# xianlopez/optical_flow

Measured on AMD Instinct MI355X. Metric: image-pairs/sec training, 384x512 batch=8 per GPU, higher is better.
Workload: dtype fp32

## Files before the change

optical_flow_amd/csrc/conv_f32.hip:

```cpp
#include "common.h"
#include "conv_dev.h"
#include "conv_narrow.h"

#include <algorithm>

namespace oflow {

template <int BM, int BN, int WAVES_M, int WAVES_N, int MODE>
__global__ __launch_bounds__(256, 2) void conv_gemm_f32(GemmArgs a) {
  constexpr int WM = BM / WAVES_M, WN = BN / WAVES_N;
  constexpr int TM = WM / 32, TN = WN / 32;
  static_assert(WAVES_M * WAVES_N == 4, "4 waves");
  static_assert(TM >= 1 && TN >= 1 && WM % 32 == 0 && WN % 32 == 0, "tile");
  constexpr bool A_KCONTIG = (MODE != MODE_WGRAD);
  constexpr int SA = BM + 4;
  constexpr int SB = BN + 4;
  constexpr int A_SLOTS = BM * BK / 4 / 256;
  constexpr int B_QUADS = BK * BN / 4;
  constexpr int B_SLOTS = (B_QUADS + 255) / 256;
  static_assert(A_SLOTS >= 1, "BM >= 64");

  static_assert(2 * BK * (SA + SB) >= 4 * 1024, "epilogue images fit LDS");
  __shared__ float smem[2 * BK * (SA + SB)];
  float (*As)[BK * SA] = reinterpret_cast<float (*)[BK * SA]>(smem);
// ... 2859 lines not shown
    const int trem = t - b * tiles_x * tiles_y;
    const int oy0 = (trem / tiles_x) * XH, ox0 = (trem % tiles_x) * TT_W;
    const int iy0 = oy0 - a.pt, ix00 = ox0 - a.pl;
#pragma unroll
    for (int j = 0; j < XS; ++j) {
      const int q = tid + NT * j;
      const int r2 = q / (CIB / 4);
      const int half = r2 & 1, s = (r2 >> 1) % KS, hy = (r2 >> 1) / KS;
      const int iy = iy0 + hy;
      const bool rok = q < XQ && xc_ok && (unsigned)iy < (unsigned)a.h;
      const int ix0 = ix00 + 8 * half + s;
      const int base = ((b * a.h + iy) * a.w + ix0) * a.lda + ci0 + 4 * xcq;
#pragma unroll
      for (int e = 0; e < 8; ++e) {
        const bool ok = rok && (unsigned)(ix0 + e) < (unsigned)a.w;
        xv[j][e] = bload4(rx, ok ? (uint32_t)((base + e * a.lda) * 4) : kOOB);
      }
    }
  };
  auto store_x = [&]() {
#pragma unroll
    for (int j = 0; j < XS; ++j) {
      const int q = tid + NT * j;
      if (q < XQ) {
        const int r2 = q / (CIB / 4);
        const int half = r2 & 1, s = (r2 >> 1) % KS, hy = (r2 >> 1) / KS;
        const int ci = 4 * xcq;
        uint4* blk = &Xs[(s * HH + hy) * CIB * 2];
#pragma unroll
        for (int c = 0; c < 4; ++c) {
          float v8[8];
#pragma unroll
          for (int e = 0; e < 8; ++e) v8[e] = (&xv[j][e].x)[c];
          bf16x8 h, m, l;
          split3x8(v8, h, m, l);
          const int idx = xrow(ci + c) * 2 + (half ^ xoct(ci + c));
          blk[idx] = __builtin_bit_cast(uint4, h);
          blk[PL + idx] = __builtin_bit_cast(uint4, m);
          blk[2 * PL + idx] = __builtin_bit_cast(uint4, l);
        }
      }
    }
  };
  const int co = co0 + wco0 + lrow;
  const bool co_ok = co < a.nb;
  const uint32_t dy_lane = (uint32_t)((8 * lk * a.ldb + co) * 4);
  const bool dy_co_full = co0 + COB <= a.nb;
  auto load_dy = [&](float (&dv)[8], int t, int kk) {
    const int b = t / (tiles_x * tiles_y);
    const int trem = t - b * tiles_x * tiles_y;
    const int oy = (trem / tiles_x) * XH + kk, ox0 = (trem % tiles_x) * TT_W;
    if (dy_co_full && oy < a.ho && ox0 + TT_W <= a.wo) {
      const int so = ((b * a.ho + oy) * a.wo + ox0) * a.ldb * 4;
#pragma unroll
      for (int e = 0; e < 8; ++e)
        dv[e] = __builtin_bit_cast(float, __builtin_amdgcn_raw_buffer_load_b32(
                                              rd, dy_lane + e * a.ldb * 4, so, 0));
      return;
    }
    const int ox = ox0 + 8 * lk;
    const bool rok = co_ok && oy < a.ho;
    const int base = ((b * a.ho + oy) * a.wo + ox) * a.ldb + co;
#pragma unroll
    for (int e = 0; e < 8; ++e) {
      const bool ok = rok && ox + e < a.wo;
      dv[e] = bload1(rd, ok ? (uint32_t)((base + e * a.ldb) * 4) : kOOB);
    }
  };

  f32x16 acc[KS];
#pragma unroll
  for (int t = 0; t < KS; ++t)
#pragma unroll
    for (int r = 0; r < 16; ++r) acc[t][r] = 0.f;
  const int a_base = xrow(wci0 + lrow) * 2 + (lk ^ xoct(wci0 + lrow));
  float colacc = 0.f;
  float dcur[8], dnext[8];

  if (steps > 0) {
    load_x(t_begin);
    load_dy(dcur, t_begin, 0);
    store_x();
  }
  __syncthreads();
  for (int i = 0; i < steps; ++i) {
    const int t = t_begin + i;
    const bool more = i + 1 < steps;
    if (more) load_x(t + 1);
#pragma unroll
    for (int kk = 0; kk < XH; ++kk) {
      if (kk + 1 < XH) load_dy(dnext, t, kk + 1);
      else if (more) load_dy(dnext, t + 1, 0);
      __builtin_amdgcn_sched_barrier(0);
      bf16x8 bh, bm, bl;
      split3x8(dcur, bh, bm, bl);
      if (do_colsum) {
#pragma unroll
        for (int e = 0; e < 8; ++e) colacc += dcur[e];
      }
      bf16x8 fa[2][NP];
      auto load_a = [&](bf16x8 (&f)[NP], int s) {
        const int xa = (s * HH + kk + wr) * CIB * 2 + a_base;
#pragma unroll
        for (int p = 0; p < NP; ++p) f[p] = __builtin_bit_cast(bf16x8, Xs[p * PL + xa]);
      };
      load_a(fa[0], 0);
#pragma unroll
      for (int s = 0; s < KS; ++s) {
          if (s + 1 < KS) load_a(fa[(s + 1) & 1], s + 1);
          __builtin_amdgcn_sched_barrier(0);
          const bf16x8 ah = fa[s & 1][0], am = fa[s & 1][1], al = fa[s & 1][2];
          f32x16 x = acc[s];
          x = __builtin_amdgcn_mfma_f32_32x32x16_bf16(al, bh, x, 0, 0, 0);
          x = __builtin_amdgcn_mfma_f32_32x32x16_bf16(ah, bl, x, 0, 0, 0);
          x = __builtin_amdgcn_mfma_f32_32x32x16_bf16(am, bm, x, 0, 0, 0);
          x = __builtin_amdgcn_mfma_f32_32x32x16_bf16(am, bh, x, 0, 0, 0);
          x = __builtin_amdgcn_mfma_f32_32x32x16_bf16(ah, bm, x, 0, 0, 0);
          acc[s] = __builtin_amdgcn_mfma_f32_32x32x16_bf16(ah, bh, x, 0, 0, 0);
          __builtin_amdgcn_sched_barrier(0);
      }
#pragma unroll
      for (int e = 0; e < 8; ++e) dcur[e] = dnext[e];
    }
    __syncthreads();
    if (more) store_x();
    __syncthreads();
  }

  float* S = a.slab + (int64_t)split * a.split_stride;
  if (do_colsum) {
    const float v = colacc + __shfl_xor(colacc, 32);
    if (lk == 0 && co < a.N) S[(int64_t)a.M * a.slab_ld + co] = v;
  }
  if (co < a.N) {
#pragma unroll
    for (int s = 0; s < KS; ++s)
#pragma unroll
      for (int r = 0; r < 16; ++r) {
        const int ci = ci0 + wci0 + (r & 3) + 8 * (r >> 2) + 4 * lk;
        if (ci < a.kc) S[((int64_t)(wr * KS + s) * a.kc + ci) * a.slab_ld + co] = acc[s][r];
      }
  }
}

__device__ __forceinline__ int wgx3b_slot(int ci, int oct) {
  return (ci >> 3) * 16 + ((2 * (ci & 7) + oct) ^ (((ci >> 3) & 3) << 1));
}

template <int CIB>
__device__ __forceinline__ int wgx3b_sw(int hx) {
  return ((hx >> 3) & 1) | (CIB == 64 ? ((hx >> 1) & 1) << 1 : 0);
}

template <int WAVES_CI, int WAVES_CO, int XH, int MI, int NP, int STG>
__device__ __forceinline__ void wgrad_x3b_body(const GemmArgs& a) {
  constexpr int NJ = 2 / MI;
  static_assert(MI * NJ == 2, "18 accumulator tiles per wave");
  static_assert(NP == 1 || NP == 3, "planes");
  static_assert(STG == 0 || STG == 1, "staging: three shifted copies / one pixel-major image");
  constexpr int NT = 64 * WAVES_CI * WAVES_CO;
  constexpr int CIB = 16 * MI * WAVES_CI, COB = 16 * NJ * WAVES_CO, KS = 3, HH = XH + KS - 1;
  static_assert(XH % 2 == 0 && (CIB == 32 || CIB == 64), "k-steps of 2 tile rows; wgx3b_sw");
  constexpr int HW = TT_W + KS - 1;
  constexpr int XQ = STG ? HH * HW * (CIB / 4) : HH * KS * 2 * (CIB / 4), XS = (XQ + NT - 1) / NT;
  constexpr int RB = CIB * 2;
  constexpr int PL = KS * HH * RB;
  constexpr int PXB = CIB * 2;
  constexpr int PLB = HH * HW * PXB, IMGB = NP * PLB;
  constexpr int LDSB = STG ? 2 * IMGB : NP * PL * 16;
  static_assert(NT / 64 * 512 * 4 <= LDSB && LDSB % 16 == 0, "epilogue images fit LDS");
  __shared__ uint4 Xs[LDSB / 16];
  char* const xlds = reinterpret_cast<char*>(Xs);

  const int tid = threadIdx.x;
  const int lane = tid & 63;
  const int wave = __builtin_amdgcn_readfirstlane(tid >> 6);
  const int wgid = xcd_remap(blockIdx.x, gridDim.x);
  const int split = wgid / a.tiles_total;
  const int tile = wgid - split * a.tiles_total;
  const int tile_co = tile % a.n_tiles;
  const int tile_ci = tile / a.n_tiles;
  const int ci0 = tile_ci * CIB, co0 = tile_co * COB;
  const int t_begin = split * a.k_per_split;
  const int t_end = min(a.K, t_begin + a.k_per_split);
  const int steps = max(0, t_end - t_begin);
  const int tiles_x = (a.wo + TT_W - 1) / TT_W, tiles_y = (a.ho + XH - 1) / XH;
  const rsrc_t rx = make_rsrc(a.A, a.a_bytes);
  const rsrc_t rd = make_rsrc(a.B, a.b_bytes);
  const int wci0 = (wave / WAVES_CO) * 16 * MI;
  const int wco0 = (wave % WAVES_CO) * 16 * NJ;
  const int l16 = lane & 15, lq = lane >> 4;

  const int xcq = tid % (CIB / 4);
  const bool xc_ok = ci0 + 4 * xcq < a.kc;
  constexpr int XE = STG ? 1 : 8;
  float4 xv[XS][XE];
  auto load_x = [&](int t) {
    const int b = t / (tiles_x * tiles_y);
    const int trem = t - b * tiles_x * tiles_y;
    const int oy0 = (trem / tiles_x) * XH, ox0 = (trem % tiles_x) * TT_W;
    const int iy0 = oy0 - a.pt, ix00 = ox0 - a.pl;
#pragma unroll
    for (int j = 0; j < XS; ++j) {
      const int q = tid + NT * j;
      if constexpr (STG == 1) {
        const int hp = q / (CIB / 4);
        const int hy = hp / HW, hx = hp - hy * HW;
        const int iy = iy0 + hy, ix = ix00 + hx;
        const bool ok = q < XQ && xc_ok && (unsigned)iy < (unsigned)a.h &&
                        (unsigned)ix < (unsigned)a.w;
        const int base = ((b * a.h + iy) * a.w + ix) * a.lda + ci0 + 4 * xcq;
        xv[j][0] = bload4(rx, ok ? (uint32_t)(base * 4) : kOOB);
      } else {
        const int r2 = q / (CIB / 4);
        const int half = r2 & 1, s = (r2 >> 1) % KS, hy = (r2 >> 1) / KS;
        const int iy = iy0 + hy;
        const bool rok = q < XQ && xc_ok && (unsigned)iy < (unsigned)a.h;
        const int ix0 = ix00 + 8 * half + s;
        const int base = ((b * a.h + iy) * a.w + ix0) * a.lda + ci0 + 4 * xcq;
#pragma unroll
        for (int e = 0; e < 8; ++e) {
          const bool ok = rok && (unsigned)(ix0 + e) < (unsigned)a.w;
          xv[j][e] = bload4(rx, ok ? (uint32_t)((base + e * a.lda) * 4) : kOOB);
        }
      }
    }
  };
  auto store_x = [&](int j, int buf) {
    const int q = tid + NT * j;
    if (XQ % NT == 0 || q < XQ) {
      if constexpr (STG == 1) {
        const int hp = q / (CIB / 4);
        const int hx = hp % HW;
        char* dst = xlds + buf * IMGB + hp * PXB + (((xcq >> 2) ^ wgx3b_sw<CIB>(hx)) << 5) +
                    8 * (xcq & 3);
        if constexpr (NP == 1) {
          *reinterpret_cast<uint2*>(dst) = pack_bf16x4(xv[j][0]);
        } else {
          uint2 h, m, l;
          split3x4(xv[j][0], h, m, l);
          *reinterpret_cast<uint2*>(dst) = h;
          *reinterpret_cast<uint2*>(dst + PLB) = m;
          *reinterpret_cast<uint2*>(dst + 2 * PLB) = l;
        }
      } else {
        const int r2 = q / (CIB / 4);
        const int half = r2 & 1, s = (r2 >> 1) % KS, hy = (r2 >> 1) / KS;
        uint4* blk = &Xs[(s * HH + hy) * RB];
#pragma unroll
        for (int c = 0; c < 4; ++c) {
          float v8[8];
#pragma unroll
          for (int e = 0; e < 8; ++e) v8[e] = (&xv[j][e].x)[c];
          const int idx = wgx3b_slot(4 * xcq + c, half);
          if constexpr (NP == 1) {
            blk[idx] = pack_bf16x8(make_float4(v8[0], v8[1], v8[2], v8[3]),
                                   make_float4(v8[4], v8[5], v8[6], v8[7]));
          } else {
            bf16x8 h, m, l;
            split3x8(v8, h, m, l);
            blk[idx] = __builtin_bit_cast(uint4, h);
            blk[PL + idx] = __builtin_bit_cast(uint4, m);
            blk[2 * PL + idx] = __builtin_bit_cast(uint4, l);
          }
        }
      }
    }
  };
  auto store_x_all = [&](int buf) {
#pragma unroll
    for (int j = 0; j < XS; ++j) store_x(j, buf);
  };
  int co[NJ];
  bool co_ok[NJ];
#pragma unroll
  for (int j = 0; j < NJ; ++j) {
    co[j] = co0 + wco0 + 16 * j + l16;
    co_ok[j] = co[j] < a.nb;
  }
  const int prow = lq >> 1, pcol = 8 * (lq & 1);
  const bool dy_co_full = co0 + COB <= a.nb;
  const uint32_t dy_lane = (uint32_t)(((prow * a.wo + pcol) * a.ldb + co0 + wco0 + l16) * 4);
  auto load_dy = [&](float (&dv)[NJ][8], int t, int kk) {
    const int b = t / (tiles_x * tiles_y);
    const int trem = t - b * tiles_x * tiles_y;
    const int oyr = (trem / tiles_x) * XH + 2 * kk, ox0 = (trem % tiles_x) * TT_W;
    if (dy_co_full && oyr + 1 < a.ho && ox0 + TT_W <= a.wo) {
      const int so = ((b * a.ho + oyr) * a.wo + ox0) * a.ldb * 4;
#pragma unroll
      for (int j = 0; j < NJ; ++j)
#pragma unroll
        for (int e = 0; e < 8; ++e)
          dv[j][e] = __builtin_bit_cast(float, __builtin_amdgcn_raw_buffer_load_b32(
                                                   rd, dy_lane + (e * a.ldb + 16 * j) * 4, so, 0));
      return;
    }
    const int oy = oyr + prow, ox = ox0 + pcol;
    const bool rok = oy < a.ho;
#pragma unroll
    for (int j = 0; j < NJ; ++j) {
      const int base = ((b * a.ho + oy) * a.wo + ox) * a.ldb + co[j];
#pragma unroll
      for (int e = 0; e < 8; ++e) {
        const bool ok = rok && co_ok[j] && ox + e < a.wo;
        dv[j][e] = bload1(rd, ok ? (uint32_t)((base + e * a.ldb) * 4) : kOOB);
      }
    }
  };

  f32x4 acc[KS * KS][MI][NJ];
#pragma unroll
  for (int t = 0; t < KS * KS; ++t)
#pragma unroll
    for (int i = 0; i < MI; ++i)
#pragma unroll
      for (int j = 0; j < NJ; ++j)
#pragma unroll
        for (int r = 0; r < 4; ++r) acc[t][i][j][r] = 0.f;
  int a_lane[MI];
#pragma unroll
  for (int i = 0; i < MI; ++i) a_lane[i] = prow * RB + wgx3b_slot(wci0 + 16 * i + l16, lq & 1);
  int a_tr[KS][2][MI];
  if constexpr (STG == 1) {
#pragma unroll
    for (int s = 0; s < KS; ++s)
#pragma unroll
      for (int h = 0; h < 2; ++h)
#pragma unroll
        for (int i = 0; i < MI; ++i) {
          const int hx = pcol + s + 4 * h + ((lane >> 2) & 3);
          a_tr[s][h][i] = (prow * HW + hx) * PXB +
                          ((((wci0 >> 4) + i) ^ wgx3b_sw<CIB>(hx)) << 5) + 8 * (lane & 3);
        }
  }
  const bool do_colsum = a.colsum && tile_ci == 0 && wci0 == 0;
  float colacc[NJ];
#pragma unroll
  for (int j = 0; j < NJ; ++j) colacc[j] = 0.f;
  float dcur[NJ][8], dnext[NJ][8];

  if (steps > 0) {
    load_x(t_begin);
    load_dy(dcur, t_begin, 0);
    store_x_all(0);
  }
  __syncthreads();
  for (int i = 0; i < steps; ++i) {
    const int t = t_begin + i;
    const bool more = i + 1 < steps;
    if (more) load_x(t + 1);
    const int buf = STG ? i & 1 : 0;
    int a_cur[KS][2][MI];
    if constexpr (STG == 1) {
#pragma unroll
      for (int s = 0; s < KS; ++s)
#pragma unroll
        for (int h = 0; h < 2; ++h)
#pragma unroll
          for (int ii = 0; ii < MI; ++ii) a_cur[s][h][ii] = a_tr[s][h][ii] + buf * IMGB;
    }
#pragma unroll
    for (int kk = 0; kk < XH / 2; ++kk) {
      if (kk + 1 < XH / 2) load_dy(dnext, t, kk + 1);
      else if (more) load_dy(dnext, t + 1, 0);
      __builtin_amdgcn_sched_barrier(0);
      bf16x8 bh[NJ], bm[NJ], bl[NJ];
#pragma unroll
      for (int j = 0; j < NJ; ++j) {
        if constexpr (NP == 1)
          bh[j] = __builtin_bit_cast(bf16x8, pack_bf16x8(make_float4(dcur[j][0], dcur[j][1], dcur[j][2], dcur[j][3]),
                                                         make_float4(dcur[j][4], dcur[j][5], dcur[j][6], dcur[j][7])));
        else
          split3x8(dcur[j], bh[j], bm[j], bl[j]);
      }
      if (do_colsum) {
#pragma unroll
        for (int j = 0; j < NJ; ++j)
#pragma unroll
          for (int e = 0; e < 8; ++e) colacc[j] += dcur[j][e];
      }
      bf16x8 fa[2][MI][NP];
      auto load_a = [&](bf16x8 (&f)[MI][NP], int tap) {
        const int r = tap / KS, s = tap % KS;
#pragma unroll
        for (int i = 0; i < MI; ++i) {
          if constexpr (STG == 1) {
#pragma unroll
            for (int p = 0; p < NP; ++p) {
              const int ro = p * PLB + (2 * kk + r) * HW * PXB;
              f[i][p] = tr_frag(xlds, a_cur[s][0][i] + ro, a_cur[s][1][i] + ro);
            }
          } else {
            const int xa = (s * HH + 2 * kk + r) * RB + a_lane[i];
#pragma unroll
            for (int p = 0; p < NP; ++p) f[i][p] = __builtin_bit_cast(bf16x8, Xs[p * PL + xa]);
          }
        }
      };
      load_a(fa[0], 0);
#pragma unroll
      for (int tap = 0; tap < KS * KS; ++tap) {
        if (tap + 1 < KS * KS) load_a(fa[(tap + 1) & 1], tap + 1);
        __builtin_amdgcn_sched_barrier(0);
#pragma unroll
        for (int i = 0; i < MI; ++i) {
          if constexpr (NP == 1) {
#pragma unroll
            for (int j = 0; j < NJ; ++j)
              acc[tap][i][j] = __builtin_amdgcn_mfma_f32_16x16x32_bf16(fa[tap & 1][i][0], bh[j],
                                                                       acc[tap][i][j], 0, 0, 0);
            continue;
          } else {
          const bf16x8 ah = fa[tap & 1][i][0], am = fa[tap & 1][i][1], al = fa[tap & 1][i][2];
#pragma unroll
          for (int j = 0; j < NJ; ++j) {
            f32x4 x = acc[tap][i][j];
            x = __builtin_amdgcn_mfma_f32_16x16x32_bf16(al, bh[j], x, 0, 0, 0);
            x = __builtin_amdgcn_mfma_f32_16x16x32_bf16(ah, bl[j], x, 0, 0, 0);
            x = __builtin_amdgcn_mfma_f32_16x16x32_bf16(am, bm[j], x, 0, 0, 0);
            x = __builtin_amdgcn_mfma_f32_16x16x32_bf16(am, bh[j], x, 0, 0, 0);
            x = __builtin_amdgcn_mfma_f32_16x16x32_bf16(ah, bm[j], x, 0, 0, 0);
            acc[tap][i][j] = __builtin_amdgcn_mfma_f32_16x16x32_bf16(ah, bh[j], x, 0, 0, 0);
          }
          }
        }
        __builtin_amdgcn_sched_barrier(0);
      }
#pragma unroll
      for (int j = 0; j < NJ; ++j)
#pragma unroll
        for (int e = 0; e < 8; ++e) dcur[j][e] = dnext[j][e];
      if constexpr (STG == 1) {
        if (more) {
#pragma unroll
          for (int j = 0; j < XS; ++j)
            if (j * (XH / 2) / XS == kk) store_x(j, buf ^ 1);
        }
        __builtin_amdgcn_sched_barrier(0);
      }
    }
    __syncthreads();
    if constexpr (STG == 0) {
      if (more) store_x_all(0);
      __syncthreads();
    }
  }

  float* S = a.slab + (int64_t)split * a.split_stride;
  if (do_colsum) {
#pragma unroll
    for (int j = 0; j < NJ; ++j) {
      float v = colacc[j] + __shfl_xor(colacc[j], 16);
      v += __shfl_xor(v, 32);
      if (lq == 0 && co[j] < a.N) S[(int64_t)a.M * a.slab_ld + co[j]] = v;
    }
  }
  constexpr int EW = 16 * NJ, LPR = 4 * NJ, RPI = 64 / LPR;
  float* E = reinterpret_cast<float*>(Xs) + wave * 512;
  const int c4 = lane % LPR, rr = lane / LPR;
  const bool vec = a.vec_ep;
#pragma unroll
  for (int tap = 0; tap < KS * KS; ++tap) {
    if (vec) {
#pragma unroll
      for (int i = 0; i < MI; ++i)
#pragma unroll
        for (int j = 0; j < NJ; ++j)
#pragma unroll
          for (int r = 0; r < 4; ++r) E[(16 * i + 4 * lq + r) * EW + 16 * j + l16] = acc[tap][i][j][r];
      __builtin_amdgcn_fence(__ATOMIC_RELEASE, "wavefront");
      __builtin_amdgcn_wave_barrier();
      __builtin_amdgcn_fence(__ATOMIC_ACQUIRE, "wavefront");
#pragma unroll
      for (int q = 0; q < 16 * MI / RPI; ++q) {
        const int row = RPI * q + rr;
        const int ci = ci0 + wci0 + row, n = co0 + wco0 + 4 * c4;
        const float4 v = *reinterpret_cast<const float4*>(&E[row * EW + 4 * c4]);
        if (ci < a.kc && n < a.N)
          *reinterpret_cast<float4*>(&S[((int64_t)tap * a.kc + ci) * a.slab_ld + n]) = v;
      }
      __builtin_amdgcn_fence(__ATOMIC_RELEASE, "wavefront");
      __builtin_amdgcn_wave_barrier();
      __builtin_amdgcn_fence(__ATOMIC_ACQUIRE, "wavefront");
    } else {
#pragma unroll
      for (int i = 0; i < MI; ++i)
#pragma unroll
        for (int j = 0; j < NJ; ++j)
#pragma unroll
          for (int r = 0; r < 4; ++r) {
            const int ci = ci0 + wci0 + 16 * i + 4 * lq + r;
            if (ci < a.kc && co[j] < a.N)
              S[((int64_t)tap * a.kc + ci) * a.slab_ld + co[j]] = acc[tap][i][j][r];
          }
    }
  }
}

template <int WAVES_CI, int WAVES_CO, int XH, int MI = 1>
__global__ __launch_bounds__(64 * WAVES_CI * WAVES_CO, 1) void conv_wgrad_tile_x3b(GemmArgs a) {
  wgrad_x3b_body<WAVES_CI, WAVES_CO, XH, MI, 3, 1>(a);
}

template <int WAVES_CI, int WAVES_CO, int XH>
__global__ __launch_bounds__(64 * WAVES_CI * WAVES_CO, 1) void conv_wgrad_tile_b16(GemmArgs a) {
  wgrad_x3b_body<WAVES_CI, WAVES_CO, XH, 1, 1, 1>(a);
}

template <int WAVES_CI, int WAVES_CO, int XH, int MI = 1>
__global__ __launch_bounds__(64 * WAVES_CI * WAVES_CO, 1) void conv_wgrad_tile_x3b_c3(GemmArgs a) {
  wgrad_x3b_body<WAVES_CI, WAVES_CO, XH, MI, 3, 0>(a);
}
template <int WAVES_CI, int WAVES_CO, int XH>
__global__ __launch_bounds__(64 * WAVES_CI * WAVES_CO, 1) void conv_wgrad_tile_b16_c3(GemmArgs a) {
  wgrad_x3b_body<WAVES_CI, WAVES_CO, XH, 1, 1, 0>(a);
}

__device__ __forceinline__ int wx3_sw(int r) { return (0x78 >> (2 * ((r >> 2) & 3))) & 3; }

template <int BM, int BN, int WAVES_M, int WAVES_N, int NP = 3>
__global__ __launch_bounds__(64 * WAVES_M * WAVES_N, NP == 1 ? 2 : 1) void conv_wgrad_x3(GemmArgs a) {
  static_assert(NP == 3 || NP == 1, "three split planes (fp32) or one (bf16)");
  constexpr int NT = 64 * WAVES_M * WAVES_N, NW = NT / 64;
  constexpr int WM = BM / WAVES_M, WN = BN / WAVES_N, SM = WM / 16, SN = WN / 16;
  static_assert(SM >= 1 && SN >= 1 && WM % 16 == 0 && WN % 16 == 0, "tile");
  constexpr int NSLOT = BM + BN, SPT = (NSLOT + NT - 1) / NT;
  constexpr int A_U4 = NP * BM * 4, B_U4 = NP * BN * 4;
  constexpr int OP_U4 = 2 * (A_U4 + B_U4), EP_U4 = NW * WM * WN * 4 / 16;
  static_assert(4 * BN * 4 <= OP_U4 * 16, "column-sum image fits LDS");
  __shared__ uint4 smem[OP_U4 > EP_U4 ? OP_U4 : EP_U4];

  const int tid = threadIdx.x;
  const int lane = tid & 63;
  const int wave = __builtin_amdgcn_readfirstlane(tid >> 6);
  const int wgid = xcd_remap(blockIdx.x, gridDim.x);
  const int split = wgid / a.tiles_total;
  const int tile = wgid - split * a.tiles_total;
  const int tile_n = tile % a.n_tiles;
  const int tile_m = tile / a.n_tiles;
  const int m0 = tile_m * BM, n0 = tile_n * BN;
  const int M = a.M;
  const int k_begin = split * a.k_per_split;
  const int k_end = min(a.K, k_begin + a.k_per_split);
  const int nchunks = k_end > k_begin ? (k_end - k_begin + BKH - 1) / BKH : 0;
  const rsrc_t rx = make_rsrc(a.A, a.a_bytes);
  const rsrc_t rd = make_rsrc(a.B, a.b_bytes);
  const bool do_colsum = a.colsum && tile_m == 0;

  bool s_isa[SPT], s_ok[SPT];
  int s_row[SPT], s_oc[SPT], s_col[SPT], s_r[SPT], s_s[SPT];
  int s_b[SPT], s_oy[SPT], s_ox[SPT];
#pragma unroll
  for (int j = 0; j < SPT; ++j) {
    const int sl = tid + NT * j;
    const bool live = sl < NSLOT;
    const bool isa = sl < BM;
    const int q = isa ? sl : sl - BM;
    const int nq = isa ? BM / 4 : BN / 4;
    const int rq = q % nq, oc = q / nq;
    s_isa[j] = isa;
    s_row[j] = 4 * rq;
    s_oc[j] = live ? oc : -1;
    if (isa) {
      const int m = m0 + 4 * rq;
      s_ok[j] = live && m < M;
      const int mm = m < M ? m : 0;
      const int tap = mm / a.kc;
      s_col[j] = mm - tap * a.kc;
      s_r[j] = tap / a.kw;
      s_s[j] = tap - s_r[j] * a.kw;
    } else {
      const int n = n0 + 4 * rq;
      s_ok[j] = live && n < a.nb;
      s_col[j] = n;
      s_r[j] = s_s[j] = 0;
    }
    const int k = k_begin + 8 * oc;
    const int hw = a.ho * a.wo;
    const int kk = k < a.K ? k : 0;
    s_b[j] = kk / hw;
    const int rem = kk - s_b[j] * hw;
    s_oy[j] = rem / a.wo;
    s_ox[j] = rem - s_oy[j] * a.wo;
  }
  float4 stg[SPT][8];
  float4 colacc = make_float4(0.f, 0.f, 0.f, 0.f);
  int kc0 = k_begin;
  auto load = [&]() {
#pragma unroll
    for (int j = 0; j < SPT; ++j) {
      int b = s_b[j], oy = s_oy[j], ox = s_ox[j];
      const int kbase = kc0 + 8 * s_oc[j];
#pragma unroll
      for (int e = 0; e < 8; ++e) {
        const bool okk = s_ok[j] && s_oc[j] >= 0 && kbase + e < k_end;
        uint32_t off = kOOB;
        if (s_isa[j]) {
          const int sy = oy * a.stride - a.pt + s_r[j], sx = ox * a.stride - a.pl + s_s[j];
          if (okk && (unsigned)sy < (unsigned)a.h && (unsigned)sx < (unsigned)a.w)
            off = (uint32_t)((((b * a.h + sy) * a.w + sx) * a.lda + s_col[j]) * 4);
          stg[j][e] = bload4(rx, off);
        } else {
          if (okk) off = (uint32_t)(((kbase + e) * a.ldb + s_col[j]) * 4);
          stg[j][e] = bload4(rd, off);
        }
        if (++ox >= a.wo) {
          ox = 0;
          if (++oy >= a.ho) {
            oy = 0;
            ++b;
          }
        }
      }
    }
  };
  auto advance = [&]() {
    kc0 += BKH;
#pragma unroll
    for (int j = 0; j < SPT; ++j) {
      s_ox[j] += BKH;
      while (s_ox[j] >= a.wo) {
        s_ox[j] -= a.wo;
        if (++s_oy[j] >= a.ho) {
          s_oy[j] = 0;
          ++s_b[j];
        }
      }
    }
  };
  auto store = [&](int buf) {
#pragma unroll
    for (int j = 0; j < SPT; ++j) {
      if (s_oc[j] < 0) continue;
      const int rows = s_isa[j] ? BM : BN;
      uint4* img = smem + (s_isa[j] ? buf * A_U4 : 2 * A_U4 + buf * B_U4);
#pragma unroll
      for (int c = 0; c < 4; ++c) {
        float v8[8];
#pragma unroll
        for (int e = 0; e < 8; ++e) v8[e] = (&stg[j][e].x)[c];
        const int row = s_row[j] + c;
        const int idx = row * 4 + (s_oc[j] ^ wx3_sw(row));
        if (NP == 1) {
          img[idx] = pack_bf16x8(make_float4(v8[0], v8[1], v8[2], v8[3]),
                                 make_float4(v8[4], v8[5], v8[6], v8[7]));
        } else {
          bf16x8 h, m, l;
          split3x8(v8, h, m, l);
          img[idx] = __builtin_bit_cast(uint4, h);
          img[(NP / 2) * rows * 4 + idx] = __builtin_bit_cast(uint4, m);
          img[(NP - 1) * rows * 4 + idx] = __builtin_bit_cast(uint4, l);
        }
      }
      if (!s_isa[j] && do_colsum) {
// ... 1196 lines not shown
  cib = wgt_cfg(d) == 0 ? 32 : 64;
  cob = wgt_cfg(d) == 0 ? 128 : 64;
}

int wgx3_cfg(const of_conv_desc* d) {
  if (!tile_ok(d)) return -1;
  if (d->cout == 64) return d->cin_p % 64 == 0 || !g_wgx3_c4 ? 2 : 4;
  return d->cout % 128 == 0 ? 0 : d->cout == 96 ? 1 : d->cout == 32 ? 3 : -1;
}
bool wgx3_ok(const of_conv_desc* d) { return wgx3_cfg(d) >= 0; }
void wgx3_blocks(const of_conv_desc* d, int& cib, int& cob) {
  const int c = wgx3_cfg(d);
  cib = c == 2 || c == 3 ? 64 : 32;
  cob = c == 0 ? 128 : c == 1 ? 96 : c == 2 || c == 4 ? 64 : 32;
}

static int g_stem_wg = 1;
bool stem_wg_ok(const of_conv_desc* d) { return g_stem_wg && stem_x3_ok(d) && d->cin == 3; }
int stem_wg_tiles(const of_conv_desc* d) {
  return d->n * (int)cdiv(d->ho, SW_TH) * (int)cdiv(d->wo, SW_TW);
}

static int g_wgrad_wgs = 4;
static int g_x3_direct = 1;
static int g_bnp_b16 = 0;

static int g_gemm_b16 = 6;
static int g_wgt_pf = 1;

enum class Fam { narrow, gemm_f32, gemm_bf16, gemm_x3, gemm_b16, tile_bf16, tile_x3, tile_b16,
                 tile_ws, stem };
enum class WFam { narrow, stem, tile_x3, tile_b16, gemm_x3, gemm_b16, tile, gemm_bf16, gemm_f32 };

Fam gemm_family(int prec, int mode) {
  if (!prec) return Fam::gemm_f32;
  if (prec == 2) return Fam::gemm_x3;
  return (g_gemm_b16 & (mode == MODE_FWD ? 1 : 2)) ? Fam::gemm_b16 : Fam::gemm_bf16;
}
Fam tile_family(const of_conv_desc* d, int prec, int mode, bool bnp = false) {
  if (prec == 2) return Fam::tile_x3;
  if (ws_ok(d, mode)) return Fam::tile_ws;
  return g_tile_b16 == 1 || (bnp && g_bnp_b16) ? Fam::tile_b16 : Fam::tile_bf16;
}
Fam fwd_family(const of_conv_desc* d, int prec, bool plain, bool stem_kernel = true) {
  if (!prec) return narrow_ok(d) && plain ? Fam::narrow : Fam::gemm_f32;
  if (tile_ok(d)) return tile_family(d, prec, MODE_FWD);
  if (stem_kernel && (prec == 2 || g_stem_bf16) && g_stem_x3 && stem_x3_ok(d)) return Fam::stem;
  return gemm_family(prec, MODE_FWD);
}
Fam dgrad_family(const of_conv_desc* d, int prec, bool bnp = false) {
  if (!prec) return narrow_ok(d) ? Fam::narrow : Fam::gemm_f32;
  return tile_ok(d) ? tile_family(d, prec, MODE_DGRAD, bnp) : gemm_family(prec, MODE_DGRAD);
}

GemmArgs plan_args(const of_conv_desc* d, const Geo& g, int mode, Fam f, bool in_place = false) {
  if (f == Fam::tile_bf16 || f == Fam::tile_x3 || f == Fam::tile_b16 || f == Fam::tile_ws)
    return tile_args(d, g, mode, f == Fam::tile_x3, f == Fam::tile_b16, f == Fam::tile_ws);
  const bool k16 = f != Fam::gemm_f32 && f != Fam::narrow;
  GemmArgs a = mode == MODE_FWD ? fwd_args(d, g, k16) : dgrad_args(d, g, k16, in_place);
  if (f == Fam::gemm_x3 || f == Fam::gemm_b16) gemm_x3_plan(a);
  return a;
}

template <int MODE>
int launch_family(Fam f, const GemmArgs& a, hipStream_t s, double flops) {
  switch (f) {
    case Fam::tile_x3: return launch<MODE>(tile_x3_launch<MODE>(a), a, s, flops);
    case Fam::tile_ws:
      return launch<MODE>(with_cfg(tile_ws_launch(a, MODE), kind(KIND_TILE_WS, MODE, 0)), a, s, flops);
    case Fam::tile_b16: return launch<MODE>(tile_b16_launch<MODE>(a), a, s, flops);
    case Fam::tile_bf16: return launch<MODE>(tile_bf16_launch<MODE>(a), a, s, flops);
    case Fam::gemm_x3: return launch<MODE>(gemm_x3_launch<MODE>(a), a, s, flops);
    case Fam::gemm_b16: return launch<MODE>(gemm_x3_launch<MODE, 1>(a), a, s, flops);
    case Fam::gemm_bf16: return launch<MODE>(gemm_bf16_launch<MODE>(a), a, s, flops);
    case Fam::gemm_f32: return launch<MODE>(gemm_f32_launch<MODE>(a), a, s, flops);
    default: return fail(OF_EINVAL, "conv: no GEMM launch for this family");
  }
}

WFam wgrad_family(const of_conv_desc* d, int prec) {
  const bool bf16 = prec == 1;
  if (narrow_ok(d)) return WFam::narrow;
  if (stem_wg_ok(d) && (!bf16 || g_stem_bf16)) return WFam::stem;
  if (prec == 2 && wgx3_ok(d)) return WFam::tile_x3;
  if (bf16 && g_wgrad_b16 && wgx3_ok(d)) return WFam::tile_b16;
  if (prec == 2 && g_wgx3_gemm) return WFam::gemm_x3;
  if (bf16 && (g_gemm_b16 & 4) && !tile_ok(d)) return WFam::gemm_b16;
  if (wgt_ok(d, bf16)) return WFam::tile;
  return bf16 ? WFam::gemm_bf16 : WFam::gemm_f32;
}

void wgrad_tiles(GemmArgs& a, const of_conv_desc* d, const Geo& g, bool x3) {
  int cib, cob;
  x3 ? wgx3_blocks(d, cib, cob) : wgt_blocks(d, cib, cob);
  a.K = d->n * (int)cdiv(d->ho, x3 ? wgx3_rows(wgx3_cfg(d)) : TT_H) * (int)cdiv(d->wo, TT_W);
  a.n_tiles = (int)cdiv(d->cout, cob);
  a.tiles_total = (int)cdiv(g.cin_p, cib) * a.n_tiles;
}

WgradPlan wgrad_plan(const of_conv_desc* d, int prec) {
  Geo g = geo(d);
  const WFam f = wgrad_family(d, prec);
  WgradPlan p;
  p.M = g.taps * g.cin_p;
  p.ldc = g.cout_p;
  p.split_stride = (int64_t)(p.M + 1) * p.ldc;
  auto slice = [&p](int units, int splits, int step = 1) {
    p.k_per_split = (int)round_up(cdiv(units, std::max(1, splits)), step);
    p.splits = (int)cdiv(units, p.k_per_split);
    return p;
  };
  if (f == WFam::stem)
    return slice(stem_wg_tiles(d), std::min(stem_wg_tiles(d), SW_WGS_PER_CU * device_cus()));
  if (f == WFam::tile_x3 || f == WFam::tile_b16 || f == WFam::tile) {
    GemmArgs t{};
    wgrad_tiles(t, d, g, f != WFam::tile);
    const int splits = std::min(t.K, device_cus() / t.tiles_total);
    return slice(t.K, f == WFam::tile ? splits : std::min(splits, t.K / g_wgx3_min_tiles));
  }
  const int K = d->n * d->ho * d->wo;
  if (f == WFam::gemm_x3 || f == WFam::gemm_b16) {
    const int tiles = (int)(cdiv(p.M, 128) * cdiv(d->cout, d->cout > 64 ? 128 : 64));
    const int splits = std::max(1, (f == WFam::gemm_b16 ? 2 : 1) * device_cus() / tiles);
    return slice(K, std::min(splits, (int)std::max<int64_t>(1, cdiv(K, 8 * BKH))), BKH);
  }
  const int bk = prec == 1 ? BKH : BK;
  const int tiles = (int)(cdiv(p.M, pick_bm(d->cout)) * cdiv(d->cout, pick_bn(d->cout)));
  const int splits = std::max(1, (g_wgrad_wgs * device_cus()) / tiles);
  return slice(K, std::min(splits, (int)std::max<int64_t>(1, cdiv(K, 8 * bk))), bk);
}
size_t wgrad_workspace(const of_conv_desc* d, int prec) {
  if (validate(d) != OF_OK) return 0;
  if (narrow_ok(d)) return narrow_wgrad_ws(d);
  const WgradPlan p = wgrad_plan(d, prec);
  return (size_t)p.splits * p.split_stride * sizeof(float);
}

template <int NP, bool FUSED = false>
constexpr Launch wgrad_stem_rec() {
  return {conv_wgrad_stem_x3<NP, FUSED>, SW_NT, NP == 1 ? KIND_STEM_WG_B16 : KIND_STEM_WG_X3,
          FUSED ? "conv_wgrad_stem_x3 fused" : "conv_wgrad_stem_x3"};
}
template <int CI, int CO, int R, int XH>
constexpr Launch wgrad_tile_x3_rec() {
  return {conv_wgrad_tile_x3<CI, CO, R, XH>, 64 * CI * CO * R, kind(KIND_TILE_X3, MODE_WGRAD, 0),
          "conv_wgrad_tile_x3"};
}
template <int STAGE, int CI, int CO, int XH, int MI = 1>
constexpr Launch wgrad_x3b_rec() {
  return {STAGE ? conv_wgrad_tile_x3b<CI, CO, XH, MI> : conv_wgrad_tile_x3b_c3<CI, CO, XH, MI>,
          64 * CI * CO, KIND_WGRAD_X3B, "conv_wgrad_tile_x3"};
}
template <int STAGE, int CI, int CO, int XH>
constexpr Launch wgrad_b16_rec() {
  return {STAGE ? conv_wgrad_tile_b16<CI, CO, XH> : conv_wgrad_tile_b16_c3<CI, CO, XH>,
          64 * CI * CO, KIND_WGRAD_B16, "conv_wgrad_tile_b16"};
}
template <int CI, int CO, int PF = 1>
constexpr Launch wgrad_tile_bf16_rec() {
  return {conv_wgrad_tile_bf16<CI, CO, PF>, 256, kind(KIND_TILE_BF16, MODE_WGRAD, 0), "conv_wgrad_tile"};
}
template <int CI, int CO>
constexpr Launch wgrad_tile_f32_rec() {
  return {conv_wgrad_tile_f32<CI, CO>, 256, kind(KIND_TILE_F32, MODE_WGRAD, 0), "conv_wgrad_tile"};
}

Launch wgrad_tile_x3_launch(int cfg) {
  static const Launch B[2][2][5] = {
      {{wgrad_x3b_rec<0, 2, 4, 8>(), wgrad_x3b_rec<0, 2, 3, 8>(), wgrad_x3b_rec<0, 4, 2, 4>(),
        wgrad_x3b_rec<0, 4, 1, 4>(), wgrad_x3b_rec<0, 2, 2, 8>()},
       {wgrad_x3b_rec<0, 1, 8, 8, 2>(), wgrad_x3b_rec<0, 1, 6, 8, 2>(), wgrad_x3b_rec<0, 2, 4, 4, 2>(),
        wgrad_x3b_rec<0, 2, 2, 4, 2>(), wgrad_x3b_rec<0, 1, 4, 8, 2>()}},
      {{wgrad_x3b_rec<1, 2, 4, 8>(), wgrad_x3b_rec<1, 2, 3, 8>(), wgrad_x3b_rec<1, 4, 2, 4>(),
        wgrad_x3b_rec<1, 4, 1, 4>(), wgrad_x3b_rec<1, 2, 2, 8>()},
       {wgrad_x3b_rec<1, 1, 8, 8, 2>(), wgrad_x3b_rec<1, 1, 6, 8, 2>(), wgrad_x3b_rec<1, 2, 4, 4, 2>(),
        wgrad_x3b_rec<1, 2, 2, 4, 2>(), wgrad_x3b_rec<1, 1, 4, 8, 2>()}}};
  static const Launch T[4] = {wgrad_tile_x3_rec<1, 4, 3, 8>(), wgrad_tile_x3_rec<1, 3, 3, 8>(),
                              wgrad_tile_x3_rec<2, 2, 3, 4>(), wgrad_tile_x3_rec<2, 1, 3, 4>()};
  const bool x3b = g_wgx3b == 2 || (g_wgx3b == 1 && cfg == 0) || cfg == 4;
  return with_cfg(x3b ? B[g_wgx3b_stage][g_wgx3b_mi - 1][cfg] : T[cfg], cfg);
}
Launch wgrad_tile_b16_launch(int cfg) {
  static const Launch T[2][5] = {
      {wgrad_b16_rec<0, 2, 4, 8>(), wgrad_b16_rec<0, 2, 3, 8>(), wgrad_b16_rec<0, 4, 2, 4>(),
       wgrad_b16_rec<0, 4, 1, 4>(), wgrad_b16_rec<0, 2, 2, 8>()},
      {wgrad_b16_rec<1, 2, 4, 8>(), wgrad_b16_rec<1, 2, 3, 8>(), wgrad_b16_rec<1, 4, 2, 4>(),
       wgrad_b16_rec<1, 4, 1, 4>(), wgrad_b16_rec<1, 2, 2, 8>()}};
  return with_cfg(T[g_wgx3b_stage][cfg], cfg);
}
Launch wgrad_tile_launch(int cfg, bool bf16) {
  static const Launch T16[2][2] = {{wgrad_tile_bf16_rec<1, 4, 0>(), wgrad_tile_bf16_rec<2, 2, 0>()},
                                   {wgrad_tile_bf16_rec<1, 4>(), wgrad_tile_bf16_rec<2, 2>()}};
  static const Launch T32[2] = {wgrad_tile_f32_rec<1, 4>(), wgrad_tile_f32_rec<2, 2>()};
  return with_cfg(bf16 ? T16[g_wgt_pf != 0][cfg / 2] : T32[cfg / 2], cfg);
}

}
}

using namespace oflow;

extern "C" {

int64_t of_conv_wfwd_elems(const of_conv_desc* d) {
  if (validate(d) != OF_OK) return -1;
  Geo g = geo(d);
  return (int64_t)g.kf * g.nf;
}

int64_t of_conv_wbwd_elems(const of_conv_desc* d) {
  if (validate(d) != OF_OK) return -1;
  Geo g = geo(d);
  return g.kd * g.nd;
}

int64_t of_conv_wfwd16_elems(const of_conv_desc* d) {
  if (validate(d) != OF_OK) return -1;
  Geo g = geo(d);
  return (int64_t)g.cout_p * g.kf16;
}

int64_t of_conv_wbwd16_elems(const of_conv_desc* d) {
  if (validate(d) != OF_OK) return -1;
  Geo g = geo(d);
  return g.kd16 * g.nd;
}

static PackEntry pack_entry(const of_conv_desc* d, const float* w, void* wf, void* wd,
                            int bf16) {
  const Geo g = geo(d);
  PackEntry E{};
  E.w = w;
  E.wf = static_cast<float*>(wf);
  E.wd = static_cast<float*>(wd);
  E.taps = g.taps;
  E.kw = d->kw;
  E.cin = d->cin;
  E.cout = d->cout;
  E.cin_p = g.cin_p;
  E.cout_p = g.cout_p;
  E.kf = g.kf;
  E.nf = g.nf;
  E.nd = g.nd;
  E.bf16 = bf16;
  E.kf16 = g.kf16;
  E.kd16 = g.kd16;
  E.pg = g.pg;
  return E;
}

static int64_t pack_work(const of_conv_desc* d, int bf16) {
  const Geo g = geo(d);
  return bf16 ? (int64_t)g.cout_p * g.kf16 + g.kd16 * g.nd : (int64_t)g.kf * g.nf + g.kd * g.nd;
}

static int64_t pack_work_many(const of_conv_desc* d, int bf16) {
  const Geo g = geo(d);
  return bf16 ? g.kd16 * g.nd : (int64_t)g.kf * g.nf + g.kd * g.nd;
}
static int64_t pack_tiles16(const of_conv_desc* d, int bf16) {
  const Geo g = geo(d);
  return bf16 ? cdiv(g.cout_p, PK_TN) * cdiv(g.kf16, PK_TK) : 0;
}

int of_conv_pack_weights_bf16(const of_conv_desc* d, const float* w_hwio, void* w16_fwd,
                              void* w16_bwd, void* stream) {
  int st = validate(d);
  if (st) return st;
  OF_CHECK_ARG(w_hwio && w16_fwd && w16_bwd, "pack bf16: NULL pointer");
  const int64_t total = pack_work(d, 1);
  OF_CHECK_ARG(total < INT32_MAX, "pack: layer too large");
  const int blocks = (int)std::min<int64_t>(cdiv(total, 256), 4096);
  hipLaunchKernelGGL(pack_one_kernel, dim3(blocks), dim3(256), 0, as_stream(stream),
                     pack_entry(d, w_hwio, w16_fwd, w16_bwd, 1), total);
  return check_launch("pack_bf16");
}

int of_conv_pack_weights(const of_conv_desc* d, const float* w_hwio, float* w_fwd,
                         float* w_bwd, void* stream) {
  int st = validate(d);
  if (st) return st;
  OF_CHECK_ARG(w_hwio && w_fwd, "pack: NULL pointer");
  Geo g = geo(d);
  hipStream_t s = as_stream(stream);
  {
    const int64_t total = (int64_t)g.kf * g.nf;
    const int blocks = (int)std::min<int64_t>(cdiv(total, 256), 4096);
    hipLaunchKernelGGL(pack_fwd_kernel, dim3(blocks), dim3(256), 0, s, w_hwio, g.taps, d->cin,
                       d->cout, g.cin_p, g.kf, g.nf, w_fwd);
    if ((st = check_launch("pack_fwd"))) return st;
  }
  if (w_bwd) {
    const int64_t total = g.kd * g.nd;
    const int blocks = (int)std::min<int64_t>(cdiv(total, 256), 4096);
    hipLaunchKernelGGL(pack_bwd_kernel, dim3(blocks), dim3(256), 0, s, w_hwio, g.pg, d->kw,
                       d->cin, d->cout, g.cout_p, g.nd, w_bwd);
    if ((st = check_launch("pack_bwd"))) return st;
  }
  return OF_OK;
}

int of_set_tuning(int key, int value) {
  if (key == 8 && value >= 0 && value <= 2) { g_stem_x3 = value; return OF_OK; }
  if (key == 7 && (value == 0 || value == 1)) { g_warp_win = value; return OF_OK; }
  if (key == 9 && value >= 0 && value <= 7) { g_corr_blk = value; return OF_OK; }
  if (key == 19 && (value == 0 || value == 1)) { g_corr_ty8 = value; return OF_OK; }
  if (key == 10 && value >= 1 && value <= 16) { g_wgrad_wgs = value; return OF_OK; }
  if (key == 11 && (value == 0 || value == 1)) { g_wgx3_c4 = value; return OF_OK; }
  if (key == 1 && value >= 1 && value <= 16) { g_split_wgs = value; return OF_OK; }
  if (key == 2 && value >= 2 && value <= 64) { g_split_min_chunks = value; return OF_OK; }
  if (key == 3 && (value == 0 || value == 1)) { g_vec_ep = value; return OF_OK; }
  if (key == 4 && value >= 0 && value <= 2) { g_wgx3b = value; return OF_OK; }
  if (key == 5 && (value == 1 || value == 2)) { g_wgx3b_mi = value; return OF_OK; }
  if (key == 6 && (value == 0 || value == 1)) { g_wgx3_gemm = value; return OF_OK; }
  if (key == 12 && value >= 0 && value <= 3) { g_tile_b16 = value; return OF_OK; }
  if (key == 13 && (value == 0 || value == 1)) { g_wgrad_b16 = value; return OF_OK; }
  if (key == 14 && (value == 0 || value == 1)) { g_stem_wg = value; return OF_OK; }
  if (key == 15 && (value == 0 || value == 1)) { g_stem_bf16 = value; return OF_OK; }
  if (key == 16 && value >= 0 && value <= 7) { g_gemm_b16 = value; return OF_OK; }
  if (key == 18 && (value == 0 || value == 1)) { g_tall16_dgrad = value; return OF_OK; }
  if (key == 17 && (value == 0 || value == 1)) { g_wgt_pf = value; return OF_OK; }
  if (key == 20 && (value == 0 || value == 1)) { g_tile16_pf = value; return OF_OK; }
  if (key == 21 && value >= 0 && value <= 3) { g_b16i_abl = value; return OF_OK; }
  if (key == 22 && (value == 0 || value == 1)) { g_b16i_direct = value; return OF_OK; }
  if (key == 23 && value >= 0 && value <= 3) { g_x3_direct = value; return OF_OK; }
  if (key == 24 && value >= 0 && value <= 2) { g_b16i_persist = value; return OF_OK; }
  if (key == 25 && value >= 0 && value <= 1000) { g_x3t_ep = value; return OF_OK; }
// ... 644 lines not shown
```

Before: 635.2.

## Carry shared input-row fragments across k-steps and add 8-wave narrow-CO wgrad variant

In the x3b weight-gradient kernel, the last tap row's LDS transpose fragments of one k-step are kept in registers and reused as the first tap row of the next k-step. This avoids redundant LDS reads when MI==1. A new NJ=1 variant doubles the CO waves (8 waves, 9 accumulator tiles per wave) and is used for the narrow-CO configurations 3 and 4. The carry adds register pressure, and the 8-wave split changes occupancy and per-block dy sharing.

```diff
diff --git a/optical_flow_amd/csrc/conv_f32.hip b/optical_flow_amd/csrc/conv_f32.hip
--- a/optical_flow_amd/csrc/conv_f32.hip
+++ b/optical_flow_amd/csrc/conv_f32.hip
@@ -3035,12 +3035,20 @@
   return ((hx >> 3) & 1) | (CIB == 64 ? ((hx >> 1) & 1) << 1 : 0);
 }
 
-template <int WAVES_CI, int WAVES_CO, int XH, int MI, int NP, int STG>
+#ifndef WGX3B_W8
+#define WGX3B_W8 1
+#endif
+#ifndef WGX3B_CARRY
+#define WGX3B_CARRY 1
+#endif
+
+template <int WAVES_CI, int WAVES_CO, int XH, int MI, int NP, int STG, int NJ = 2 / MI,
+          bool CARRY = false>
 __device__ __forceinline__ void wgrad_x3b_body(const GemmArgs& a) {
-  constexpr int NJ = 2 / MI;
-  static_assert(MI * NJ == 2, "18 accumulator tiles per wave");
+  static_assert(MI * NJ == 2 || (MI == 1 && NJ == 1), "18 or 9 accumulator tiles per wave");
   static_assert(NP == 1 || NP == 3, "planes");
   static_assert(STG == 0 || STG == 1, "staging: three shifted copies / one pixel-major image");
+  static_assert(!CARRY || STG == 1, "carried fragments: the pixel-major image");
   constexpr int NT = 64 * WAVES_CI * WAVES_CO;
   constexpr int CIB = 16 * MI * WAVES_CI, COB = 16 * NJ * WAVES_CO, KS = 3, HH = XH + KS - 1;
   static_assert(XH % 2 == 0 && (CIB == 32 || CIB == 64), "k-steps of 2 tile rows; wgx3b_sw");
@@ -3242,6 +3250,7 @@
 #pragma unroll
           for (int ii = 0; ii < MI; ++ii) a_cur[s][h][ii] = a_tr[s][h][ii] + buf * IMGB;
     }
+    bf16x8 carry[KS][MI][NP];
 #pragma unroll
     for (int kk = 0; kk < XH / 2; ++kk) {
       if (kk + 1 < XH / 2) load_dy(dnext, t, kk + 1);
@@ -3270,8 +3279,13 @@
           if constexpr (STG == 1) {
 #pragma unroll
             for (int p = 0; p < NP; ++p) {
+              if (CARRY && kk > 0 && r == 0) {
+                f[i][p] = carry[s][i][p];
+                continue;
+              }
               const int ro = p * PLB + (2 * kk + r) * HW * PXB;
               f[i][p] = tr_frag(xlds, a_cur[s][0][i] + ro, a_cur[s][1][i] + ro);
+              if (CARRY && r == KS - 1 && kk + 1 < XH / 2) carry[s][i][p] = f[i][p];
             }
           } else {
             const int xa = (s * HH + 2 * kk + r) * RB + a_lane[i];
@@ -3380,9 +3394,23 @@
   }
 }
 
+template <int XH, int MI>
+constexpr bool wgx3b_carry() {
+  return WGX3B_CARRY && XH / 2 > 1 && MI == 1;
+}
+
 template <int WAVES_CI, int WAVES_CO, int XH, int MI = 1>
 __global__ __launch_bounds__(64 * WAVES_CI * WAVES_CO, 1) void conv_wgrad_tile_x3b(GemmArgs a) {
-  wgrad_x3b_body<WAVES_CI, WAVES_CO, XH, MI, 3, 1>(a);
+  wgrad_x3b_body<WAVES_CI, WAVES_CO, XH, MI, 3, 1, 2 / MI, wgx3b_carry<XH, MI>()>(a);
+}
+
+template <int WAVES_CI, int WAVES_CO, int XH>
+__global__ __launch_bounds__(64 * WAVES_CI * WAVES_CO, 1) void conv_wgrad_tile_x3b_n1(GemmArgs a) {
+  wgrad_x3b_body<WAVES_CI, WAVES_CO, XH, 1, 3, 1, 1, wgx3b_carry<XH, 1>()>(a);
+}
+template <int WAVES_CI, int WAVES_CO, int XH>
+__global__ __launch_bounds__(64 * WAVES_CI * WAVES_CO, 1) void conv_wgrad_tile_x3b_n1_c3(GemmArgs a) {
+  wgrad_x3b_body<WAVES_CI, WAVES_CO, XH, 1, 3, 0, 1>(a);
 }
 
 template <int WAVES_CI, int WAVES_CO, int XH>
@@ -4885,6 +4913,15 @@
           64 * CI * CO, KIND_WGRAD_X3B, "conv_wgrad_tile_x3"};
 }
 template <int STAGE, int CI, int CO, int XH>
+constexpr Launch wgrad_x3b_n1_rec() {
+#if WGX3B_W8
+  return {STAGE ? conv_wgrad_tile_x3b_n1<CI, 2 * CO, XH> : conv_wgrad_tile_x3b_n1_c3<CI, 2 * CO, XH>,
+          128 * CI * CO, KIND_WGRAD_X3B, "conv_wgrad_tile_x3"};
+#else
+  return wgrad_x3b_rec<STAGE, CI, CO, XH>();
+#endif
+}
+template <int STAGE, int CI, int CO, int XH>
 constexpr Launch wgrad_b16_rec() {
   return {STAGE ? conv_wgrad_tile_b16<CI, CO, XH> : conv_wgrad_tile_b16_c3<CI, CO, XH>,
           64 * CI * CO, KIND_WGRAD_B16, "conv_wgrad_tile_b16"};
@@ -4901,11 +4938,11 @@
 Launch wgrad_tile_x3_launch(int cfg) {
   static const Launch B[2][2][5] = {
       {{wgrad_x3b_rec<0, 2, 4, 8>(), wgrad_x3b_rec<0, 2, 3, 8>(), wgrad_x3b_rec<0, 4, 2, 4>(),
-        wgrad_x3b_rec<0, 4, 1, 4>(), wgrad_x3b_rec<0, 2, 2, 8>()},
+        wgrad_x3b_n1_rec<0, 4, 1, 4>(), wgrad_x3b_n1_rec<0, 2, 2, 8>()},
        {wgrad_x3b_rec<0, 1, 8, 8, 2>(), wgrad_x3b_rec<0, 1, 6, 8, 2>(), wgrad_x3b_rec<0, 2, 4, 4, 2>(),
         wgrad_x3b_rec<0, 2, 2, 4, 2>(), wgrad_x3b_rec<0, 1, 4, 8, 2>()}},
       {{wgrad_x3b_rec<1, 2, 4, 8>(), wgrad_x3b_rec<1, 2, 3, 8>(), wgrad_x3b_rec<1, 4, 2, 4>(),
-        wgrad_x3b_rec<1, 4, 1, 4>(), wgrad_x3b_rec<1, 2, 2, 8>()},
+        wgrad_x3b_n1_rec<1, 4, 1, 4>(), wgrad_x3b_n1_rec<1, 2, 2, 8>()},
        {wgrad_x3b_rec<1, 1, 8, 8, 2>(), wgrad_x3b_rec<1, 1, 6, 8, 2>(), wgrad_x3b_rec<1, 2, 4, 4, 2>(),
         wgrad_x3b_rec<1, 2, 2, 4, 2>(), wgrad_x3b_rec<1, 1, 4, 8, 2>()}}};
   static const Launch T[4] = {wgrad_tile_x3_rec<1, 4, 3, 8>(), wgrad_tile_x3_rec<1, 3, 3, 8>(),
```

After: 638.7, median of 6. Within noise of the previous version (+0.6%).
